# peleiden/rl-rubiks

Hardware: AMD Instinct MI355X
Metric: MCTS node expansions/sec, depth-20 scrambles (higher is better)
Workload: dtype f32 (f16x3 split: three f16 MFMA products per layer, fp32 accumulate); 1 GPU; 1024 depth-20 MCTS trees/GPU, c=0.6, graph search, max_states 175000, pool 8x1024, fc_small weights/fc_small_r1; trees_per_gpu=1024, max_states=175000, scramble_depth=20, parallelism=scramble-sharded x1

## Files before the change

rl-rubiks_amd/csrc/rubiks_net.hip:

```cpp
#include <atomic>

#include <type_traits>

#include "rubiks_common.h"
#include "rubiks_netmath.h"

namespace rubiks {

constexpr int kOH = 480;

__device__ __forceinline__ float act_apply(float x, int act, float alpha) {
    if (act == RC_ACT_RELU) return fmaxf(x, 0.f);
    if (act == RC_ACT_ELU) return x > 0.f ? x : alpha * (__expf(x) - 1.f);
    return x;
}


typedef __attribute__((ext_vector_type(8))) __bf16 bf16x8;
typedef __attribute__((ext_vector_type(8))) _Float16 f16x8;
typedef __attribute__((ext_vector_type(16))) float f32x16;

constexpr int kMfCols = 128;
constexpr int kMfPitch = 976;
constexpr int kMfWaves = 8;
constexpr int kMfTile = 32;
constexpr int kMfSub = 1;

template <int ACT, bool F16>
__global__ __launch_bounds__(kMfWaves * kWave) void k_first_layer_mfma(const u8 *__restrict__ soa, size_t n, size_t stride,
                                                                     const uint4 *__restrict__ w1, const float *__restrict__ bias,
                                                                     uint4 *__restrict__ out, u32 H, u32 rows_per_block,
                                                                     float alpha) {
    extern __shared__ __attribute__((aligned(256))) unsigned char lds[];
    unsigned char *wslice = lds;
    const u32 tid = threadIdx.x, wave = tid >> 6, lane = tid & 63;
    uint4 *onehot = reinterpret_cast<uint4 *>(lds + kMfCols * kMfPitch);
    const u32 col_tiles = H / kMfCols;
    const u32 ct = blockIdx.x % col_tiles, rg = blockIdx.x / col_tiles;
    const size_t row_lo = (size_t)rg * rows_per_block;
    if (row_lo >= n) return;
    const size_t row_hi = (row_lo + rows_per_block < n) ? row_lo + rows_per_block : n;

    {
        constexpr int kPer = kMfCols * 60 / (kMfWaves * kWave), kBatch = 5;
#pragma unroll
        for (int b0 = 0; b0 < kPer; b0 += kBatch) {
            uint4 tmp[kBatch];
#pragma unroll
            for (int t = 0; t < kBatch; ++t) {
                const u32 i = tid + (b0 + t) * (kMfWaves * kWave);
                tmp[t] = w1[(size_t)(ct * kMfCols + i / 60) * 60 + i % 60];
            }
#pragma unroll
            for (int t = 0; t < kBatch; ++t) {
                const u32 i = tid + (b0 + t) * (kMfWaves * kWave);
                const u32 g = i / 60, slot = (g & 3) * 32 + (g >> 2);
                *reinterpret_cast<uint4 *>(wslice + slot * kMfPitch + (i % 60) * 16) = tmp[t];
            }
        }
    }
    if (tid < 9) {
        u32 w[4] = {0, 0, 0, 0};
        const u32 one = F16 ? 0x3c00u : 0x3f80u;
        if (tid < 8) w[tid >> 1] = (tid & 1) ? one << 16 : one;
        onehot[tid] = make_uint4(w[0], w[1], w[2], w[3]);
    }
    const u32 r = lane & 31, h = lane >> 5;
    float b[4];
#pragma unroll
    for (int c = 0; c < 4; ++c) b[c] = bias[ct * kMfCols + 4 * r + c];
    __syncthreads();

    const u32 off_a = h ? 8u : 0u, off_c = h ? 16u : 8u;
    constexpr size_t kStep = (size_t)kMfWaves * kMfSub * kMfTile;
    for (size_t t0 = row_lo + (size_t)wave * kMfSub * kMfTile; t0 < row_hi; t0 += kStep) {
        u32 pk[kMfSub][5];
#pragma unroll
        for (int u = 0; u < kMfSub; ++u) {
            const size_t row = t0 + (size_t)u * kMfTile + r;
            const u8 *p = soa + (row < n ? row : n - 1);
            u32 raw[kPlanes];
#pragma unroll
            for (int j = 0; j < kPlanes; ++j) raw[j] = p[(size_t)j * stride];
#pragma unroll
            for (int q = 0; q < 5; ++q)
                pk[u][q] = (raw[4 * q] & 31u) | (raw[4 * q + 1] & 31u) << 8 | (raw[4 * q + 2] & 31u) << 16 | (raw[4 * q + 3] & 31u) << 24;
        }
        auto code = [&](int u, int j) -> u32 { return (pk[u][j >> 2] >> (8 * (j & 3))) & 0xffu; };
        f32x16 acc[kMfSub][4];
#pragma unroll
        for (int u = 0; u < kMfSub; ++u)
#pragma unroll
            for (int c = 0; c < 4; ++c)
#pragma unroll
                for (int i = 0; i < 16; ++i) acc[u][c][i] = b[c];
        auto a_frag = [&](int u, int ks) -> uint4 {
            const int m2 = ks / 3, ph = ks % 3;
            const u32 pos = ph == 0 ? code(u, 2 * m2) - off_a : ph == 1 ? (h ? code(u, 2 * m2 + 1) : code(u, 2 * m2) - 16u)
                                                                         : code(u, 2 * m2 + 1) - off_c;
            return onehot[min(pos, 8u)];
        };
        const unsigned char *bbase = wslice + r * kMfPitch + 16 * h;
        uint4 a_cur[kMfSub], b_cur[4];
#pragma unroll
        for (int u = 0; u < kMfSub; ++u) a_cur[u] = a_frag(u, 0);
#pragma unroll
        for (int c = 0; c < 4; ++c) b_cur[c] = *reinterpret_cast<const uint4 *>(bbase + c * 32 * kMfPitch);
#pragma unroll
        for (int ks = 0; ks < 30; ++ks) {
            uint4 a_nxt[kMfSub], b_nxt[4] = {b_cur[0], b_cur[1], b_cur[2], b_cur[3]};
#pragma unroll
            for (int u = 0; u < kMfSub; ++u) a_nxt[u] = a_cur[u];
            if (ks + 1 < 30) {
#pragma unroll
                for (int c = 0; c < 4; ++c) b_nxt[c] = *reinterpret_cast<const uint4 *>(bbase + c * 32 * kMfPitch + 32 * (ks + 1));
#pragma unroll
                for (int u = 0; u < kMfSub; ++u) a_nxt[u] = a_frag(u, ks + 1);
            }
            __builtin_amdgcn_sched_barrier(0);
#pragma unroll
            for (int c = 0; c < 4; ++c)
#pragma unroll
                for (int u = 0; u < kMfSub; ++u) {
                    if (F16)
                        acc[u][c] = __builtin_amdgcn_mfma_f32_32x32x16_f16(__builtin_bit_cast(f16x8, a_cur[u]),
                                                                           __builtin_bit_cast(f16x8, b_cur[c]), acc[u][c], 0, 0, 0);
                    else
                        acc[u][c] = __builtin_amdgcn_mfma_f32_32x32x16_bf16(__builtin_bit_cast(bf16x8, a_cur[u]),
                                                                            __builtin_bit_cast(bf16x8, b_cur[c]), acc[u][c], 0, 0, 0);
                }
            __builtin_amdgcn_sched_barrier(0);
#pragma unroll
            for (int u = 0; u < kMfSub; ++u) a_cur[u] = a_nxt[u];
#pragma unroll
            for (int c = 0; c < 4; ++c) b_cur[c] = b_nxt[c];
        }
        uint2 *out2 = reinterpret_cast<uint2 *>(out);
#pragma unroll
        for (int u = 0; u < kMfSub; ++u)
#pragma unroll
            for (int i = 0; i < 16; ++i) {
                const size_t row = t0 + (size_t)u * kMfTile + (i & 3) + 8 * (i >> 2) + 4 * h;
                const uint2 v = make_uint2(pack_bf16(act_apply(acc[u][0][i], ACT, alpha), act_apply(acc[u][1][i], ACT, alpha)),
                                           pack_bf16(act_apply(acc[u][2][i], ACT, alpha), act_apply(acc[u][3][i], ACT, alpha)));
                if (row < n) out2[row * (H / 4) + ct * (kMfCols / 4) + r] = v;
            }
    }
}

typedef __attribute__((ext_vector_type(4))) float f32x4;
constexpr int kHeadK = 1024, kHeadSteps = kHeadK / 32, kHeadMaxOut = 16;

// ... 360 lines not shown
__global__ __launch_bounds__(kMfWaves * kWave) void k_first_layer_split(const u8 *__restrict__ soa, size_t n, size_t stride,
                                                                      const uint4 *__restrict__ w_hi, const uint4 *__restrict__ w_lo,
                                                                      const float *__restrict__ bias, u32 *__restrict__ out, u32 H,
                                                                      u32 rows_per_block, float alpha, int *__restrict__ range_flag) {
    extern __shared__ __attribute__((aligned(256))) unsigned char lds[];
    constexpr int kTables = 2;
    bool out_of_range = false;
    unsigned char *wslice = lds;
    const u32 tid = threadIdx.x, lane = tid & 63;
    const u32 wave = __builtin_amdgcn_readfirstlane(tid >> 6);
    uint4 *onehot = reinterpret_cast<uint4 *>(lds + kTables * kSpCols * kMfPitch);
    const u32 col_tiles = H / kSpCols;
    const u32 ct = blockIdx.x % col_tiles, rg = blockIdx.x / col_tiles;
    const size_t row_lo = (size_t)rg * rows_per_block;
    if (row_lo >= n) return;
    const size_t row_hi = (row_lo + rows_per_block < n) ? row_lo + rows_per_block : n;
    {
        constexpr int kBatch = 5, kPer = kTables * kSpCols * 60 / (kMfWaves * kWave) / kBatch * kBatch;
#pragma unroll
        for (int b0 = 0; b0 < kPer; b0 += kBatch) {
            uint4 tmp[kBatch];
#pragma unroll
            for (int t = 0; t < kBatch; ++t) {
                const u32 i = tid + (b0 + t) * (kMfWaves * kWave), tbl = i / (kSpCols * 60), j = i % (kSpCols * 60);
                tmp[t] = (tbl ? w_lo : w_hi)[(size_t)(ct * kSpCols + j / 60) * 60 + j % 60];
            }
#pragma unroll
            for (int t = 0; t < kBatch; ++t) {
                const u32 i = tid + (b0 + t) * (kMfWaves * kWave), tbl = i / (kSpCols * 60), j = i % (kSpCols * 60);
                const u32 g = j / 60, slot = (g & 1) * 32 + (g >> 1);
                *reinterpret_cast<uint4 *>(wslice + (tbl * kSpCols + slot) * kMfPitch + (j % 60) * 16) = tmp[t];
            }
        }
        static_assert(kPer * kMfWaves * kWave == kTables * kSpCols * 60, "the staging loop covers the slices exactly");
    }
    if (tid < 9 * kTables) {
        u32 w[4] = {0, 0, 0, 0};
        const u32 p = tid % 9, one = tid < 9 ? kHalfOne : kHalfScaleInv;
        if (p < 8) w[p >> 1] = (p & 1) ? one << 16 : one;
        onehot[tid] = make_uint4(w[0], w[1], w[2], w[3]);
    }
    const u32 r = lane & 31, h = lane >> 5;
    float b[2];
#pragma unroll
    for (int c = 0; c < 2; ++c) b[c] = bias[ct * kSpCols + 2 * r + c];
    __syncthreads();

    const u32 off_a = h ? 8u : 0u, off_c = h ? 16u : 8u;
    constexpr size_t kStep = (size_t)kMfWaves * kSpSub * kMfTile;
    const u32 n_pass = (u32)((row_hi - row_lo + kStep - 1) / kStep);
    for (u32 pass = 0; pass < n_pass; ++pass) {
        const size_t t0 = row_lo + (size_t)pass * kStep + (size_t)wave * kSpSub * kMfTile;
        if (t0 >= row_hi) break;
        u32 pk[kSpSub][5];
#pragma unroll
        for (int u = 0; u < kSpSub; ++u) {
            const size_t row = t0 + (size_t)u * kMfTile + r;
            const u8 *p = soa + (row < n ? row : n - 1);
            u32 raw[kPlanes];
#pragma unroll
            for (int j = 0; j < kPlanes; ++j) raw[j] = p[(size_t)j * stride];
#pragma unroll
            for (int q = 0; q < 5; ++q)
                pk[u][q] = (raw[4 * q] & 31u) | (raw[4 * q + 1] & 31u) << 8 | (raw[4 * q + 2] & 31u) << 16 | (raw[4 * q + 3] & 31u) << 24;
        }
        auto code = [&](int u, int j) -> u32 { return (pk[u][j >> 2] >> (8 * (j & 3))) & 0xffu; };
        f32x16 acc[kSpSub][2];
#pragma unroll
        for (int u = 0; u < kSpSub; ++u)
#pragma unroll
            for (int c = 0; c < 2; ++c)
#pragma unroll
                for (int i = 0; i < 16; ++i) acc[u][c][i] = b[c];
#pragma unroll 1
        for (int tbl = 0; tbl < kTables; ++tbl) {
            const uint4 *frag = onehot + 9 * tbl;
            const unsigned char *bbase = wslice + ((size_t)tbl * kSpCols + r) * kMfPitch + 16 * h;
            auto a_frag = [&](int u, int ks) -> uint4 {
                const int m2 = ks / 3, ph = ks % 3;
                const u32 pos = ph == 0 ? code(u, 2 * m2) - off_a : ph == 1 ? (h ? code(u, 2 * m2 + 1) : code(u, 2 * m2) - 16u)
                                                                             : code(u, 2 * m2 + 1) - off_c;
                return frag[min(pos, 8u)];
            };
            uint4 a_cur[kSpSub], b_cur[2];
#pragma unroll
            for (int u = 0; u < kSpSub; ++u) a_cur[u] = a_frag(u, 0);
#pragma unroll
            for (int c = 0; c < 2; ++c) b_cur[c] = *reinterpret_cast<const uint4 *>(bbase + c * 32 * kMfPitch);
#pragma unroll
            for (int ks = 0; ks < 30; ++ks) {
                uint4 a_nxt[kSpSub], b_nxt[2] = {b_cur[0], b_cur[1]};
#pragma unroll
                for (int u = 0; u < kSpSub; ++u) a_nxt[u] = a_cur[u];
                if (ks + 1 < 30) {
#pragma unroll
                    for (int c = 0; c < 2; ++c) b_nxt[c] = *reinterpret_cast<const uint4 *>(bbase + c * 32 * kMfPitch + 32 * (ks + 1));
#pragma unroll
                    for (int u = 0; u < kSpSub; ++u) a_nxt[u] = a_frag(u, ks + 1);
                }
                __builtin_amdgcn_sched_barrier(0);
#pragma unroll
                for (int c = 0; c < 2; ++c)
#pragma unroll
                    for (int u = 0; u < kSpSub; ++u)
                        acc[u][c] = __builtin_amdgcn_mfma_f32_32x32x16_f16(__builtin_bit_cast(f16x8, a_cur[u]),
                                                                           __builtin_bit_cast(f16x8, b_cur[c]), acc[u][c], 0, 0, 0);
                __builtin_amdgcn_sched_barrier(0);
#pragma unroll
                for (int u = 0; u < kSpSub; ++u) a_cur[u] = a_nxt[u];
#pragma unroll
                for (int c = 0; c < 2; ++c) b_cur[c] = b_nxt[c];
            }
        }
        const size_t lim = row_hi < n ? row_hi : n;
        u32 *o_hi = out + t0 * (size_t)H + (ct * kSpCols) / 2;
        u32 *o_lo = o_hi + H / 2;
        if (t0 + (size_t)kSpSub * kMfTile <= lim) {
            u32 off = 4 * h * H + r;
#pragma unroll
            for (int u = 0; u < kSpSub; ++u)
#pragma unroll
                for (int i = 0; i < 16; ++i) {
                    const float y0 = act_value<ACT>(acc[u][0][i], alpha), y1 = act_value<ACT>(acc[u][1][i], alpha);
                    out_of_range |= !(fabsf(y0) <= 65504.0f) || !(fabsf(y1) <= 65504.0f);
                    const SplitPair sp = split_pair(y0, y1);
                    o_hi[off] = sp.hi;
                    o_lo[off] = sp.lo;
                    off += ((i & 3) == 3 ? 5u : 1u) * H;
                }
        } else {
#pragma unroll
            for (int u = 0; u < kSpSub; ++u)
#pragma unroll
                for (int i = 0; i < 16; ++i) {
                    const size_t row = t0 + (size_t)u * kMfTile + (i & 3) + 8 * (i >> 2) + 4 * h;
                    const float y0 = act_value<ACT>(acc[u][0][i], alpha), y1 = act_value<ACT>(acc[u][1][i], alpha);
                    if (row < lim) {
                        out_of_range |= !(fabsf(y0) <= 65504.0f) || !(fabsf(y1) <= 65504.0f);
                        const SplitPair sp = split_pair(y0, y1);
                        u32 *orow = out + row * H;
                        orow[(ct * kSpCols) / 2 + r] = sp.hi;
                        orow[H / 2 + (ct * kSpCols) / 2 + r] = sp.lo;
                    }
                }
        }
    }
    if (range_flag && out_of_range) atomicOr(range_flag, 1);
}

constexpr int kGaCols = 64, kGaRows = 480;
#ifndef RUBIKS_GATHER_ABLATE
#define RUBIKS_GATHER_ABLATE 0
#endif
typedef float f32x2 __attribute__((ext_vector_type(2)));

template <int ACT, int WAVES, int C, bool MAP = false>
__global__ __launch_bounds__(WAVES * kWave) void k_first_layer_gather(const u8 *__restrict__ soa, size_t n, size_t stride,
                                                                     const float4 *__restrict__ w_rows, const float *__restrict__ bias,
                                                                     unsigned char *__restrict__ out, u32 H, u32 rows_per_block, float alpha,
                                                                     int *__restrict__ range_flag, const u32 *__restrict__ rows_dev,
                                                                     const int *__restrict__ src_map) {
    static_assert(C == 4 || C == 8, "4 or 8 columns per lane");
    constexpr int R = C / 4;
    constexpr u32 kLanes = kGaCols / C;
    constexpr u32 kStates = kWave / kLanes;
    extern __shared__ __attribute__((aligned(256))) unsigned char lds[];
    const u32 tid = threadIdx.x, lane = tid & 63;
    const u32 wave = __builtin_amdgcn_readfirstlane(tid >> 6);
    const u32 col_tiles = H / kGaCols, ct = blockIdx.x % col_tiles, rg = blockIdx.x / col_tiles;
    const u32 last_state = (u32)(n - 1);
    if (MAP) {
        n = min((size_t)*rows_dev, n);
        const u32 per_group = (u32)ceil_div(n, (size_t)(gridDim.x / col_tiles)), unit = per_group < WAVES * kStates ? kStates : WAVES * kStates;
        rows_per_block = (per_group + unit - 1) / unit * unit;
    }
    const size_t row_lo = (size_t)rg * rows_per_block;
    if (row_lo >= n) return;
    const size_t row_hi = (row_lo + rows_per_block < n) ? row_lo + rows_per_block : n;
    {
        constexpr u32 kChunks = kGaRows * (kGaCols / 4), kThreads = WAVES * kWave, kBatch = 4;
        for (u32 i0 = tid; i0 < kChunks; i0 += kBatch * kThreads) {
            float4 tmp[kBatch];
#pragma unroll
            for (u32 b = 0; b < kBatch; ++b) {
                const u32 i = i0 + b * kThreads;
                if (i < kChunks) tmp[b] = w_rows[(size_t)(i >> 4) * (H / 4) + ct * (kGaCols / 4) + (i & 15)];
            }
#pragma unroll
            for (u32 b = 0; b < kBatch; ++b) {
                const u32 i = i0 + b * kThreads;
                if (i < kChunks) reinterpret_cast<float4 *>(lds)[i] = tmp[b];
            }
        }
    }
    const u32 u = lane % kLanes, sub = lane / kLanes;
    const u32 col = ct * kGaCols + C * u;
    float4 b4[R];
#pragma unroll
    for (int r = 0; r < R; ++r) b4[r] = *reinterpret_cast<const float4 *>(bias + col + 4 * r);
    bool out_of_range = false;
    const __amdgpu_buffer_rsrc_t planes = __builtin_amdgcn_make_buffer_rsrc((void *)soa, 0, (int)(u32)(kPlanes * stride), 0x00020000);
    const u32 last = (u32)(n - 1), pitch = (u32)stride;
    auto codes_of = [&](size_t t, u32 (&c)[kPlanes]) {
        u32 tv = t < n ? (u32)t : last;
        if (MAP) tv = min((u32)src_map[tv], last_state);
#pragma unroll
        for (int j = 0; j < kPlanes; ++j) c[j] = (RUBIKS_GATHER_ABLATE & 4) ? (tv + j) % 24u : (u32)__builtin_amdgcn_raw_buffer_load_b8(planes, tv, (u32)j * pitch, 0);
    };
    const u32 base0 = u * (4 * C), base1 = u * (4 * C) + 11 * 24 * (kGaCols * 4);
    __syncthreads();
    constexpr size_t kStep = (size_t)WAVES * kStates;
    size_t t = row_lo + (size_t)wave * kStates + sub;
    u32 code[kPlanes], code_next[kPlanes];
    codes_of(t, code);
    for (size_t t0 = row_lo + (size_t)wave * kStates; t0 < row_hi; t0 += kStep, t += kStep) {
        const bool more = t0 + kStep < row_hi;
        f32x2 acc[2 * R];
#pragma unroll
        for (int r = 0; r < R; ++r) acc[2 * r] = f32x2{b4[r].x, b4[r].y}, acc[2 * r + 1] = f32x2{b4[r].z, b4[r].w};
        constexpr int kBatch = 10 / R;
#pragma unroll
        for (int part = 0; part < kPlanes / kBatch; ++part) {
            float4 v[kBatch][R];
#pragma unroll
            for (int i = 0; i < kBatch; ++i) {
                const int j = part * kBatch + i;
                const u32 at = (code[j] << 8) + (j < 11 ? base0 : base1);
                const unsigned char *rowp = lds + at + (j < 11 ? j : j - 11) * 24 * (kGaCols * 4);
#pragma unroll
                for (int r = 0; r < R; ++r)
                    v[i][r] = (RUBIKS_GATHER_ABLATE & 2) ? make_float4(__uint_as_float(at), 1.f, 2.f, 3.f) : *reinterpret_cast<const float4 *>(rowp + 16 * r);
            }
            __builtin_amdgcn_sched_barrier(0);
            if (part == 0 && more) codes_of(t + kStep, code_next);
            __builtin_amdgcn_sched_barrier(0);
#pragma unroll
            for (int i = 0; i < kBatch; ++i)
#pragma unroll
                for (int r = 0; r < R; ++r) {
                    acc[2 * r] += f32x2{v[i][r].x, v[i][r].y};
                    acc[2 * r + 1] += f32x2{v[i][r].z, v[i][r].w};
                }
            __builtin_amdgcn_sched_barrier(0);
        }
        bool bad = false;
        SplitPair sp[2 * R];
#pragma unroll
        for (int p = 0; p < 2 * R; ++p) {
            if (!(RUBIKS_GATHER_ABLATE & 8)) acc[p] = act_value2<ACT>(acc[p], alpha);
            bad |= !(fabsf(acc[p].x) <= 65504.0f);
            bad |= !(fabsf(acc[p].y) <= 65504.0f);
            sp[p] = split_pair(acc[p].x, acc[p].y);
        }
        const bool live = (RUBIKS_GATHER_ABLATE & 1) ? (t < row_hi && acc[0].x == 1.2345e-30f) : t < row_hi;
        unsigned char *orow = out + t * ((size_t)H * 4);
        if (C == 8) {
            if (live) {
                out_of_range |= bad;
                *reinterpret_cast<uint4 *>(orow + (size_t)col * 2) = make_uint4(sp[0].hi, sp[1].hi, sp[2 * R - 2].hi, sp[2 * R - 1].hi);
                *reinterpret_cast<uint4 *>(orow + ((size_t)H + col) * 2) = make_uint4(sp[0].lo, sp[1].lo, sp[2 * R - 2].lo, sp[2 * R - 1].lo);
            }
        } else {
            constexpr int kSwapPairs = 0xB1;
            const u32 n_hi0 = (u32)__builtin_amdgcn_mov_dpp((int)sp[0].hi, kSwapPairs, 0xF, 0xF, true), n_hi1 = (u32)__builtin_amdgcn_mov_dpp((int)sp[1].hi, kSwapPairs, 0xF, 0xF, true);
            const u32 n_lo0 = (u32)__builtin_amdgcn_mov_dpp((int)sp[0].lo, kSwapPairs, 0xF, 0xF, true), n_lo1 = (u32)__builtin_amdgcn_mov_dpp((int)sp[1].lo, kSwapPairs, 0xF, 0xF, true);
            if (live) {
                out_of_range |= bad;
                const bool odd = lane & 1u;
                const uint4 both = odd ? make_uint4(n_lo0, n_lo1, sp[0].lo, sp[1].lo) : make_uint4(sp[0].hi, sp[1].hi, n_hi0, n_hi1);
                *reinterpret_cast<uint4 *>(orow + (odd ? (size_t)H + col - 4 : (size_t)col) * 2) = both;
            }
        }
        if (more) {
#pragma unroll
            for (int j = 0; j < kPlanes; ++j) code[j] = code_next[j];
        }
    }
    if (range_flag && out_of_range) atomicOr(range_flag, 1);
}

extern "C" int rc_oh_split_f16(const int8_t *soa, size_t n, size_t stride, uint16_t *out, rc_stream_t stream) {
    if (n == 0) return RC_OK;
    RC_CHECK_SOA(soa, n, stride);
    RC_REQUIRE(out != nullptr, RC_ERR_NULL);
    RC_REQUIRE(aligned16(out), RC_ERR_ALIGN);
    hipLaunchKernelGGL(k_oh_split_f16, dim3(grid_for(n * (2 * kOH / 8), kBlock, 256 * 16)), dim3(kBlock), 0, (hipStream_t)stream,
                       (const u8 *)soa, n, stride, (uint4 *)out);
    return launch_status();
}

extern "C" int rc_split_act_f16(const float *c, const float *c_corr, float corr_scale, size_t n_rows, size_t n_cols, const float *bias,
                                int activation, float alpha, uint16_t *out_hi_lo, float *out_f32, rc_stream_t stream) {
    if (n_rows == 0 || n_cols == 0) return RC_OK;
    RC_REQUIRE(c && bias && (out_hi_lo || out_f32), RC_ERR_NULL);
    RC_REQUIRE(aligned16(c) && aligned16(c_corr) && aligned16(bias) && aligned16(out_hi_lo) && aligned16(out_f32) && n_cols % 8 == 0, RC_ERR_ALIGN);
    RC_REQUIRE(activation >= RC_ACT_NONE && activation <= RC_ACT_ELU, RC_ERR_RANGE);
    const dim3 grid(grid_for(n_rows * (n_cols / 8), kBlock, 256 * 16)), block(kBlock);
    hipStream_t s = (hipStream_t)stream;
#define RC_LAUNCH_SPLIT(ACT)                                                                                                  \
    hipLaunchKernelGGL(k_split_act<ACT>, grid, block, 0, s, (const float4 *)c, (const float4 *)c_corr, corr_scale, n_rows, n_cols, \
                       (const float4 *)bias, alpha,                                                                            \
                       (uint4 *)out_hi_lo, (float4 *)out_f32)
    if (activation == RC_ACT_ELU) RC_LAUNCH_SPLIT(RC_ACT_ELU);
    else if (activation == RC_ACT_RELU) RC_LAUNCH_SPLIT(RC_ACT_RELU);
    else RC_LAUNCH_SPLIT(RC_ACT_NONE);
#undef RC_LAUNCH_SPLIT
    return launch_status();
}

static int split_reduce(const float *partials, size_t partial_stride, int n_partials, int n_corr, size_t n_rows, size_t n_cols,
                        const float *bias, const uint16_t *residual_hi_lo, int activation, float alpha, const float *post_scale,
                        const float *post_shift, uint16_t *out_hi_lo, float *out_f32, int32_t *range_flag, const uint32_t *rows_dev,
                        rc_stream_t stream) {
    if (n_rows == 0 || n_cols == 0) return RC_OK;
    RC_REQUIRE(partials && bias && (out_hi_lo || out_f32), RC_ERR_NULL);
    RC_REQUIRE((post_scale == nullptr) == (post_shift == nullptr), RC_ERR_NULL);
    RC_REQUIRE(aligned16(partials) && aligned16(bias) && aligned16(residual_hi_lo) && aligned16(post_scale) && aligned16(post_shift) &&
                   aligned16(out_hi_lo) && aligned16(out_f32) && n_cols % 8 == 0 && partial_stride % 4 == 0, RC_ERR_ALIGN);
    RC_REQUIRE(activation >= RC_ACT_NONE && activation <= RC_ACT_ELU && n_partials >= 1 && n_partials <= 64 && n_corr >= 0 &&
                   n_corr <= n_partials && (n_partials == 1 || partial_stride >= n_rows * n_cols), RC_ERR_RANGE);
    const dim3 grid(grid_for(n_rows * (n_cols / 8), kBlock, 256 * 16)), block(kBlock);
    hipStream_t s = (hipStream_t)stream;
#define RC_LAUNCH_RED(ACT)                                                                                                       \
    hipLaunchKernelGGL(k_split_reduce<ACT>, grid, block, 0, s, (const float4 *)partials, partial_stride / 4, n_partials, n_corr, n_rows, \
                       n_cols, (const float4 *)bias, (const uint4 *)residual_hi_lo, alpha, (const float4 *)post_scale,                \
                       (const float4 *)post_shift, (uint4 *)out_hi_lo, (float4 *)out_f32, (int *)range_flag, rows_dev)
    if (activation == RC_ACT_ELU) RC_LAUNCH_RED(RC_ACT_ELU);
    else if (activation == RC_ACT_RELU) RC_LAUNCH_RED(RC_ACT_RELU);
    else RC_LAUNCH_RED(RC_ACT_NONE);
#undef RC_LAUNCH_RED
    return launch_status();
}

extern "C" int rc_split_reduce_f16(const float *partials, size_t partial_stride, int n_partials, int n_corr, size_t n_rows, size_t n_cols,
                                   const float *bias, const uint16_t *residual_hi_lo, int activation, float alpha, const float *post_scale,
                                   const float *post_shift, uint16_t *out_hi_lo, float *out_f32, int32_t *range_flag, rc_stream_t stream) {
    return split_reduce(partials, partial_stride, n_partials, n_corr, n_rows, n_cols, bias, residual_hi_lo, activation, alpha, post_scale,
                        post_shift, out_hi_lo, out_f32, range_flag, nullptr, stream);
}

extern "C" int rc_split_reduce_rows_f16(const float *partials, size_t partial_stride, int n_partials, int n_corr, size_t n_rows, size_t n_cols,
                                        const float *bias, const uint16_t *residual_hi_lo, int activation, float alpha,
                                        const float *post_scale, const float *post_shift, uint16_t *out_hi_lo, float *out_f32,
                                        int32_t *range_flag, const uint32_t *rows_dev, rc_stream_t stream) {
    RC_REQUIRE(rows_dev != nullptr, RC_ERR_NULL);
    return split_reduce(partials, partial_stride, n_partials, n_corr, n_rows, n_cols, bias, residual_hi_lo, activation, alpha, post_scale,
                        post_shift, out_hi_lo, out_f32, range_flag, rows_dev, stream);
}

static int head_split(const float *c, const float *c_corr, float corr_scale, size_t n, size_t K, const float *bias_h, int activation,
                      float alpha, const float *w, const float *bias_o, size_t n_out, float *out, const uint32_t *rows_dev,
                      const int32_t *src_map, rc_stream_t stream) {
    if (n == 0) return RC_OK;
    RC_REQUIRE(c && bias_h && w && bias_o && out && (rows_dev == nullptr) == (src_map == nullptr), RC_ERR_NULL);
    RC_REQUIRE(aligned16(c) && aligned16(c_corr) && aligned16(bias_h) && aligned16(w), RC_ERR_ALIGN);
    RC_REQUIRE((K == 512 || K == 1024) && n_out >= 1 && n_out <= (size_t)kHeadMaxOut && activation >= RC_ACT_NONE && activation <= RC_ACT_ELU,
               RC_ERR_RANGE);
    const unsigned grid = grid_for(ceil_div(n, (size_t)16) * kBlock, kBlock, 256 * 4);
    hipStream_t s = (hipStream_t)stream;
#define RC_LAUNCH_HS(ACT, KB, MAP)                                                                                             \
    hipLaunchKernelGGL((k_head_split<ACT, KB, MAP>), dim3(grid), dim3(kBlock), 0, s, (const float4 *)c, (const float4 *)c_corr, corr_scale, \
                       n, (const float4 *)bias_h, alpha, (const float4 *)w, bias_o, (u32)n_out, out, rows_dev, src_map)
#define RC_LAUNCH_HS_K(ACT)                                     \
    do {                                                        \
        if (rows_dev) {                                         \
            if (K == 1024) RC_LAUNCH_HS(ACT, 16, true);         \
            else RC_LAUNCH_HS(ACT, 8, true);                    \
        } else if (K == 1024) RC_LAUNCH_HS(ACT, 16, false);     \
        else RC_LAUNCH_HS(ACT, 8, false);                       \
    } while (0)
    if (activation == RC_ACT_ELU) RC_LAUNCH_HS_K(RC_ACT_ELU);
    else if (activation == RC_ACT_RELU) RC_LAUNCH_HS_K(RC_ACT_RELU);
    else RC_LAUNCH_HS_K(RC_ACT_NONE);
#undef RC_LAUNCH_HS_K
#undef RC_LAUNCH_HS
    return launch_status();
}

extern "C" int rc_head_split_f32(const float *c, const float *c_corr, float corr_scale, size_t n, size_t K, const float *bias_h,
                                 int activation, float alpha, const float *w, const float *bias_o, size_t n_out, float *out,
                                 rc_stream_t stream) {
    return head_split(c, c_corr, corr_scale, n, K, bias_h, activation, alpha, w, bias_o, n_out, out, nullptr, nullptr, stream);
}

extern "C" int rc_head_split_rows_f32(const float *c, const float *c_corr, float corr_scale, size_t n, size_t K, const float *bias_h,
                                      int activation, float alpha, const float *w, const float *bias_o, size_t n_out, float *out,
                                      const uint32_t *rows_dev, const int32_t *src_map, rc_stream_t stream) {
    RC_REQUIRE(rows_dev && src_map, RC_ERR_NULL);
    return head_split(c, c_corr, corr_scale, n, K, bias_h, activation, alpha, w, bias_o, n_out, out, rows_dev, src_map, stream);
}

extern "C" int rc_first_layer_split_f16(const int8_t *soa, size_t n, size_t stride, const uint16_t *w_hi, const uint16_t *w_lo,
                                        const float *bias, uint16_t *out_hi_lo, size_t H, int activation, float alpha,
                                        rc_stream_t stream) {
    return rc_first_layer_split_flag_f16(soa, n, stride, w_hi, w_lo, bias, out_hi_lo, H, activation, alpha, nullptr, stream);
}

extern "C" int rc_first_layer_split_flag_f16(const int8_t *soa, size_t n, size_t stride, const uint16_t *w_hi, const uint16_t *w_lo,
                                             const float *bias, uint16_t *out_hi_lo, size_t H, int activation, float alpha,
                                             int32_t *range_flag, rc_stream_t stream) {
    if (n == 0) return RC_OK;
    RC_CHECK_SOA(soa, n, stride);
    RC_REQUIRE(w_hi && w_lo && bias && out_hi_lo, RC_ERR_NULL);
    RC_REQUIRE(aligned16(w_hi) && aligned16(w_lo) && aligned16(out_hi_lo), RC_ERR_ALIGN);
    RC_REQUIRE(H >= (size_t)kSpCols && H % kSpCols == 0 && activation >= RC_ACT_NONE && activation <= RC_ACT_ELU, RC_ERR_RANGE);
    const u32 col_tiles = (u32)(H / kSpCols);
    u32 row_groups = (256 + col_tiles - 1) / col_tiles;
    constexpr u32 kRowsPerPass = kMfWaves * kSpSub * kMfTile;
    const size_t per_group = ceil_div(n, row_groups);
    u32 rows_per_block = (u32)round_up(per_group, per_group < kRowsPerPass ? (size_t)kSpSub * kMfTile : (size_t)kRowsPerPass);
    row_groups = (u32)ceil_div(n, rows_per_block);
    const size_t lds_bytes = (size_t)2 * kSpCols * kMfPitch + 2 * 9 * 16;
    const dim3 grid(col_tiles * row_groups), block(kMfWaves * kWave);
    hipStream_t s = (hipStream_t)stream;
#define RC_LAUNCH_SP(ACT)                                                                                             \
    do {                                                                                                              \
        static std::atomic<unsigned long long> attr_set{0};                                                           \
        int dev_ = 0;                                                                                                 \
        (void)hipGetDevice(&dev_);                                                                                    \
        if (!((attr_set.load(std::memory_order_acquire) >> (dev_ & 63)) & 1ull)) {                                     \
            hipError_t e = hipFuncSetAttribute((const void *)k_first_layer_split<ACT>, hipFuncAttributeMaxDynamicSharedMemorySize, \
                                               (int)lds_bytes);                                                       \
            if (e != hipSuccess) return hip_rc(e);                                                                    \
            attr_set.fetch_or(1ull << (dev_ & 63), std::memory_order_release);                                        \
        }                                                                                                             \
        hipLaunchKernelGGL((k_first_layer_split<ACT>), grid, block, lds_bytes, s, (const u8 *)soa, n, stride, (const uint4 *)w_hi, \
                           (const uint4 *)w_lo, bias, (u32 *)out_hi_lo, (u32)H, rows_per_block, alpha, (int *)range_flag); \
    } while (0)
    if (activation == RC_ACT_ELU) RC_LAUNCH_SP(RC_ACT_ELU);
    else if (activation == RC_ACT_RELU) RC_LAUNCH_SP(RC_ACT_RELU);
    else RC_LAUNCH_SP(RC_ACT_NONE);
#undef RC_LAUNCH_SP
    return launch_status();
}

static int first_layer_gather(const int8_t *soa, size_t n, size_t stride, const float *w_rows, const float *bias, uint16_t *out_hi_lo,
                              size_t H, int activation, float alpha, int32_t *range_flag, const uint32_t *rows_dev, const int32_t *src_map,
                              int form, rc_stream_t stream) {
    if (n == 0) return RC_OK;
    RC_CHECK_SOA(soa, n, stride);
    RC_REQUIRE(w_rows && bias && out_hi_lo && (rows_dev == nullptr) == (src_map == nullptr), RC_ERR_NULL);
    RC_REQUIRE(form >= 0 && form <= 2, RC_ERR_RANGE);
    RC_REQUIRE(aligned16(w_rows) && aligned16(bias) && aligned16(out_hi_lo), RC_ERR_ALIGN);
    RC_REQUIRE(H >= (size_t)kGaCols && H % kGaCols == 0 && H < (1u << 24) && activation >= RC_ACT_NONE && activation <= RC_ACT_ELU, RC_ERR_RANGE);
    RC_REQUIRE(stride * kPlanes < (1ull << 32), RC_ERR_RANGE);
    const u32 col_tiles = (u32)(H / kGaCols);
    const size_t lds_bytes = (size_t)kGaRows * kGaCols * 4;
    hipStream_t s = (hipStream_t)stream;
    const bool wide = form ? form == 2 : n * col_tiles > (size_t)5000 * 64;
    const u32 waves = wide ? 8 : 16, states = wide ? 8 : 4;
    u32 row_groups = (256 + col_tiles - 1) / col_tiles;
    const u32 rows_per_pass = waves * states;
    const size_t per_group = ceil_div(n, (size_t)row_groups);
    const u32 rows_per_block = (u32)round_up(per_group, per_group < rows_per_pass ? (size_t)states : (size_t)rows_per_pass);
    row_groups = (u32)ceil_div(n, (size_t)rows_per_block);
    const dim3 grid(col_tiles * row_groups);
#define RC_LAUNCH_GA(ACT, WAVES, C, MAP)                                                                                 \
    do {                                                                                                              \
        static std::atomic<unsigned long long> attr_set{0};                                                           \
        int dev_ = 0;                                                                                                 \
        (void)hipGetDevice(&dev_);                                                                                    \
        if (!((attr_set.load(std::memory_order_acquire) >> (dev_ & 63)) & 1ull)) {                                     \
            hipError_t e = hipFuncSetAttribute((const void *)k_first_layer_gather<ACT, WAVES, C, MAP>,                \
                                               hipFuncAttributeMaxDynamicSharedMemorySize, (int)lds_bytes);           \
            if (e != hipSuccess) return hip_rc(e);                                                                    \
            attr_set.fetch_or(1ull << (dev_ & 63), std::memory_order_release);                                        \
        }                                                                                                             \
        hipLaunchKernelGGL((k_first_layer_gather<ACT, WAVES, C, MAP>), grid, dim3(WAVES * kWave), lds_bytes, s, (const u8 *)soa, n, stride, \
                           (const float4 *)w_rows, bias, (unsigned char *)out_hi_lo, (u32)H, rows_per_block, alpha, (int *)range_flag,  \
                           rows_dev, src_map);                                                                          \
    } while (0)
#define RC_LAUNCH_GA_ACT(ACT)                              \
    do {                                                   \
        if (rows_dev) {                                    \
            if (wide) RC_LAUNCH_GA(ACT, 8, 8, true);       \
            else RC_LAUNCH_GA(ACT, 16, 4, true);           \
        } else if (wide) RC_LAUNCH_GA(ACT, 8, 8, false);   \
        else RC_LAUNCH_GA(ACT, 16, 4, false);              \
    } while (0)
    if (activation == RC_ACT_ELU) RC_LAUNCH_GA_ACT(RC_ACT_ELU);
    else if (activation == RC_ACT_RELU) RC_LAUNCH_GA_ACT(RC_ACT_RELU);
    else RC_LAUNCH_GA_ACT(RC_ACT_NONE);
#undef RC_LAUNCH_GA_ACT
#undef RC_LAUNCH_GA
    return launch_status();
}

extern "C" int rc_first_layer_gather_f16(const int8_t *soa, size_t n, size_t stride, const float *w_rows, const float *bias,
                                         uint16_t *out_hi_lo, size_t H, int activation, float alpha, int32_t *range_flag,
                                         rc_stream_t stream) {
    return first_layer_gather(soa, n, stride, w_rows, bias, out_hi_lo, H, activation, alpha, range_flag, nullptr, nullptr, 0, stream);
}

extern "C" int rc_first_layer_gather_rows_f16(const int8_t *soa, size_t n, size_t stride, const float *w_rows, const float *bias,
                                              uint16_t *out_hi_lo, size_t H, int activation, float alpha, int32_t *range_flag,
                                              const uint32_t *rows_dev, const int32_t *src_map, int form, rc_stream_t stream) {
    return first_layer_gather(soa, n, stride, w_rows, bias, out_hi_lo, H, activation, alpha, range_flag, rows_dev, src_map, form, stream);
}

extern "C" int rc_adi_targets(const float *values, const uint8_t *child_solved, const uint8_t *state_solved, size_t n,
                              size_t depth, float win_reward, int fix_mode, int64_t *policy_target, float *value_target,
                              rc_stream_t stream) {
    if (n == 0) return RC_OK;
    RC_REQUIRE(values && child_solved && policy_target && value_target, RC_ERR_NULL);
    RC_REQUIRE(fix_mode >= 0 && fix_mode <= 2 && depth > 0, RC_ERR_RANGE);
    RC_REQUIRE(fix_mode != 1 || state_solved != nullptr, RC_ERR_NULL);
    hipLaunchKernelGGL(k_adi_targets, dim3(grid_for(n)), dim3(kBlock), 0, (hipStream_t)stream, values, child_solved,
                       state_solved, n, depth, win_reward, fix_mode, (long long *)policy_target, value_target);
    return launch_status();
}
```

Baseline: 14.17 million node expansions/s.

## Software-pipeline the wide first-layer gather across passes with triple-buffered codes

Rewrites the C==8 path of the first-layer gather kernel. Cubie codes are fetched two passes ahead through a rotating set of three code buffers, and the first LDS row reads of the next pass overlap the current accumulation. Lanes are remapped so each lane reads two 16-byte slices and swaps halves via DPP, allowing a single buffer store per output half. The wide launch also moves from 8 to 12 waves, and the weight staging loop is restructured to unroll fully. This aims to hide global code-load and LDS latency, at the cost of more registers and higher occupancy pressure.

```diff
diff --git a/rl-rubiks_amd/csrc/rubiks_net.hip b/rl-rubiks_amd/csrc/rubiks_net.hip
--- a/rl-rubiks_amd/csrc/rubiks_net.hip
+++ b/rl-rubiks_amd/csrc/rubiks_net.hip
@@ -1,3 +1,4 @@
+#include <utility>
 #include <atomic>
 
 #include <type_traits>
@@ -664,7 +665,26 @@
 #ifndef RUBIKS_GATHER_ABLATE
 #define RUBIKS_GATHER_ABLATE 0
 #endif
+constexpr int kGaWideWaves = 12, kGaAhead = 4;
 typedef float f32x2 __attribute__((ext_vector_type(2)));
+typedef float f32x4 __attribute__((ext_vector_type(4)));
+typedef u32 u32x4 __attribute__((ext_vector_type(4)));
+#define RC_GA_PLANES(X) X(0) X(1) X(2) X(3) X(4) X(5) X(6) X(7) X(8) X(9) X(10) X(11) X(12) X(13) X(14) X(15) X(16) X(17) X(18) X(19)
+struct GaCodes {
+#define RC_GA_FIELD(j) u32 c##j;
+    RC_GA_PLANES(RC_GA_FIELD)
+#undef RC_GA_FIELD
+    template <int J> __device__ __forceinline__ u32 &at() {
+        static_assert(J >= 0 && J < kPlanes, "one code per cubie");
+#define RC_GA_PICK(j) if constexpr (J == j) return c##j; else
+        RC_GA_PLANES(RC_GA_PICK) return c0;
+#undef RC_GA_PICK
+    }
+    template <int J> __device__ __forceinline__ u32 at() const { return const_cast<GaCodes *>(this)->template at<J>(); }
+};
+#define RC_INLINE __attribute__((always_inline))
+template <class F, int... I> __device__ __forceinline__ void static_for_each(F &&f, std::integer_sequence<int, I...>) { (f(std::integral_constant<int, I>{}), ...); }
+template <int N, class F> __device__ __forceinline__ void static_for(F &&f) { static_for_each(f, std::make_integer_sequence<int, N>{}); }
 
 template <int ACT, int WAVES, int C, bool MAP = false>
 __global__ __launch_bounds__(WAVES * kWave) void k_first_layer_gather(const u8 *__restrict__ soa, size_t n, size_t stride,
@@ -673,7 +693,6 @@
                                                                      int *__restrict__ range_flag, const u32 *__restrict__ rows_dev,
                                                                      const int *__restrict__ src_map) {
     static_assert(C == 4 || C == 8, "4 or 8 columns per lane");
-    constexpr int R = C / 4;
     constexpr u32 kLanes = kGaCols / C;
     constexpr u32 kStates = kWave / kLanes;
     extern __shared__ __attribute__((aligned(256))) unsigned char lds[];
@@ -690,89 +709,185 @@
     if (row_lo >= n) return;
     const size_t row_hi = (row_lo + rows_per_block < n) ? row_lo + rows_per_block : n;
     {
-        constexpr u32 kChunks = kGaRows * (kGaCols / 4), kThreads = WAVES * kWave, kBatch = 4;
-        for (u32 i0 = tid; i0 < kChunks; i0 += kBatch * kThreads) {
+        constexpr u32 kChunks = kGaRows * (kGaCols / 4), kThreads = WAVES * kWave, kRounds = kChunks / kThreads, kBatch = 5;
+        const float4 *src = w_rows + ct * (kGaCols / 4);
+        const auto chunk = [&](u32 i) { return src[(size_t)(i >> 4) * (H / 4) + (i & 15)]; };
+#pragma unroll
+        for (u32 r0 = 0; r0 < kRounds; r0 += kBatch) {
             float4 tmp[kBatch];
 #pragma unroll
-            for (u32 b = 0; b < kBatch; ++b) {
-                const u32 i = i0 + b * kThreads;
-                if (i < kChunks) tmp[b] = w_rows[(size_t)(i >> 4) * (H / 4) + ct * (kGaCols / 4) + (i & 15)];
-            }
-#pragma unroll
-            for (u32 b = 0; b < kBatch; ++b) {
-                const u32 i = i0 + b * kThreads;
-                if (i < kChunks) reinterpret_cast<float4 *>(lds)[i] = tmp[b];
-            }
-        }
+            for (u32 b = 0; b < kBatch; ++b)
+                if (r0 + b < kRounds) tmp[b] = chunk(tid + (r0 + b) * kThreads);
+#pragma unroll
+            for (u32 b = 0; b < kBatch; ++b)
+                if (r0 + b < kRounds) reinterpret_cast<float4 *>(lds)[tid + (r0 + b) * kThreads] = tmp[b];
+        }
+        if (kChunks % kThreads != 0 && tid < kChunks % kThreads) reinterpret_cast<float4 *>(lds)[tid + kRounds * kThreads] = chunk(tid + kRounds * kThreads);
     }
     const u32 u = lane % kLanes, sub = lane / kLanes;
-    const u32 col = ct * kGaCols + C * u;
-    float4 b4[R];
-#pragma unroll
-    for (int r = 0; r < R; ++r) b4[r] = *reinterpret_cast<const float4 *>(bias + col + 4 * r);
     bool out_of_range = false;
-    const __amdgpu_buffer_rsrc_t planes = __builtin_amdgcn_make_buffer_rsrc((void *)soa, 0, (int)(u32)(kPlanes * stride), 0x00020000);
-    const u32 last = (u32)(n - 1), pitch = (u32)stride;
-    auto codes_of = [&](size_t t, u32 (&c)[kPlanes]) {
-        u32 tv = t < n ? (u32)t : last;
-        if (MAP) tv = min((u32)src_map[tv], last_state);
-#pragma unroll
-        for (int j = 0; j < kPlanes; ++j) c[j] = (RUBIKS_GATHER_ABLATE & 4) ? (tv + j) % 24u : (u32)__builtin_amdgcn_raw_buffer_load_b8(planes, tv, (u32)j * pitch, 0);
-    };
-    const u32 base0 = u * (4 * C), base1 = u * (4 * C) + 11 * 24 * (kGaCols * 4);
-    __syncthreads();
+    const u32 last = (u32)(n - 1);
     constexpr size_t kStep = (size_t)WAVES * kStates;
     size_t t = row_lo + (size_t)wave * kStates + sub;
-    u32 code[kPlanes], code_next[kPlanes];
-    codes_of(t, code);
-    for (size_t t0 = row_lo + (size_t)wave * kStates; t0 < row_hi; t0 += kStep, t += kStep) {
-        const bool more = t0 + kStep < row_hi;
-        f32x2 acc[2 * R];
-#pragma unroll
-        for (int r = 0; r < R; ++r) acc[2 * r] = f32x2{b4[r].x, b4[r].y}, acc[2 * r + 1] = f32x2{b4[r].z, b4[r].w};
-        constexpr int kBatch = 10 / R;
-#pragma unroll
-        for (int part = 0; part < kPlanes / kBatch; ++part) {
-            float4 v[kBatch][R];
-#pragma unroll
-            for (int i = 0; i < kBatch; ++i) {
-                const int j = part * kBatch + i;
-                const u32 at = (code[j] << 8) + (j < 11 ? base0 : base1);
-                const unsigned char *rowp = lds + at + (j < 11 ? j : j - 11) * 24 * (kGaCols * 4);
-#pragma unroll
-                for (int r = 0; r < R; ++r)
-                    v[i][r] = (RUBIKS_GATHER_ABLATE & 2) ? make_float4(__uint_as_float(at), 1.f, 2.f, 3.f) : *reinterpret_cast<const float4 *>(rowp + 16 * r);
-            }
-            __builtin_amdgcn_sched_barrier(0);
-            if (part == 0 && more) codes_of(t + kStep, code_next);
-            __builtin_amdgcn_sched_barrier(0);
-#pragma unroll
-            for (int i = 0; i < kBatch; ++i)
-#pragma unroll
-                for (int r = 0; r < R; ++r) {
-                    acc[2 * r] += f32x2{v[i][r].x, v[i][r].y};
-                    acc[2 * r + 1] += f32x2{v[i][r].z, v[i][r].w};
+    if constexpr (C == 8) {
+        constexpr int kAhead = kGaAhead;
+        const u32 p = (u ^ sub) & 1u, slot = u ^ (8u * p);
+        const u32 lane0 = 16u * slot;
+        const u32 col_k = ct * kGaCols + 4 * slot, col_s = ct * kGaCols + 4 * (slot ^ 8u);
+        const float4 bias_k = *reinterpret_cast<const float4 *>(bias + col_k), bias_s = *reinterpret_cast<const float4 *>(bias + col_s);
+        const u32 row_bytes = H * 4, out_at = sub * row_bytes + (ct * kGaCols + 32u * p + 4u * (u & 6u)) * 2;
+        const bool odd = u & 1u;
+        const auto row_of = [&](size_t ahead) RC_INLINE {
+            const size_t tt = t + ahead * kStep;
+            return tt < n ? (u32)tt : last;
+        };
+        const auto request = [&](u32 tv, GaCodes &c) RC_INLINE {
+            static_for<kPlanes>([&](auto jc) RC_INLINE {
+                constexpr int j = decltype(jc)::value;
+                c.template at<j>() = (RUBIKS_GATHER_ABLATE & 4) ? (tv + j) % 24u : (u32)(soa + (size_t)j * stride)[tv];
+            });
+        };
+        typedef const f32x4 __attribute__((address_space(3))) *SliceRow;
+        u32 first0 = (u32)(size_t)(__attribute__((address_space(3))) unsigned char *)lds + lane0, first1 = first0 + 11 * 24 * (kGaCols * 4);
+        u32 to_second = (lane0 ^ 128u) - lane0;
+        asm("" : "+v"(first0), "+v"(first1), "+v"(to_second));
+        const auto read_row = [&](const GaCodes &c, auto jc, f32x4(&v)[2]) RC_INLINE {
+            constexpr int j = decltype(jc)::value;
+            constexpr u32 imm = (u32)(j < 11 ? j : j - 11) * 24 * (kGaCols * 4);
+            u32 at0 = (c.template at<j>() << 8) + (j < 11 ? first0 : first1);
+            asm("" : "+v"(at0));
+            u32 at1 = at0 + to_second;
+            asm("" : "+v"(at1));
+            if (RUBIKS_GATHER_ABLATE & 2) {
+                v[0] = v[1] = f32x4{__uint_as_float(at0 + at1), 1.f, 2.f, 3.f};
+            } else {
+                v[0] = *(SliceRow)(size_t)(at0 + imm);
+                v[1] = *(SliceRow)(size_t)(at1 + imm);
+            }
+        };
+        const bool any = row_lo + (size_t)wave * kStates < row_hi;
+        GaCodes code_a, code_b, code_c;
+        u32 map_next = 0;
+        if (any) {
+            if (MAP) {
+                request(min((u32)src_map[row_of(0)], last_state), code_a);
+                request(min((u32)src_map[row_of(1)], last_state), code_b);
+                map_next = (u32)src_map[row_of(2)];
+            } else {
+                request(row_of(0), code_a);
+                request(row_of(1), code_b);
+            }
+        }
+        __syncthreads();
+        if (!any) return;
+        f32x4 head[kAhead][2];
+        static_for<kAhead>([&](auto ic) RC_INLINE { read_row(code_a, ic, head[decltype(ic)::value]); });
+        size_t t0 = row_lo + (size_t)wave * kStates;
+        const auto pass = [&](const GaCodes &cur, const GaCodes &nxt, GaCodes &far) RC_INLINE {
+            if (MAP) {
+                const u32 state = min(map_next, last_state);
+                map_next = (u32)src_map[row_of(3)];
+                request(state, far);
+            } else {
+                request(row_of(2), far);
+            }
+            f32x2 acc[4] = {f32x2{bias_k.x, bias_k.y}, f32x2{bias_k.z, bias_k.w}, f32x2{bias_s.x, bias_s.y}, f32x2{bias_s.z, bias_s.w}};
+            f32x4 v[kPlanes + kAhead][2];
+#pragma unroll
+            for (int i = 0; i < kAhead; ++i) v[i][0] = head[i][0], v[i][1] = head[i][1];
+            static_for<kPlanes>([&](auto jc) RC_INLINE {
+                constexpr int j = decltype(jc)::value, ja = j + kAhead;
+                if constexpr (ja < kPlanes) read_row(cur, std::integral_constant<int, ja>{}, v[ja]);
+                else read_row(nxt, std::integral_constant<int, ja - kPlanes>{}, v[ja]);
+                __builtin_amdgcn_sched_barrier(0);
+                acc[0] += v[j][0].xy;
+                acc[1] += v[j][0].zw;
+                acc[2] += v[j][1].xy;
+                acc[3] += v[j][1].zw;
+                __builtin_amdgcn_sched_barrier(0);
+            });
+#pragma unroll
+            for (int i = 0; i < kAhead; ++i) head[i][0] = v[kPlanes + i][0], head[i][1] = v[kPlanes + i][1];
+            bool bad = false;
+            SplitPair sp[4];
+#pragma unroll
+            for (int q = 0; q < 4; ++q) {
+                if (!(RUBIKS_GATHER_ABLATE & 8)) acc[q] = act_value2<ACT>(acc[q], alpha);
+                bad |= !(fabsf(acc[q].x) <= 65504.0f);
+                bad |= !(fabsf(acc[q].y) <= 65504.0f);
+                sp[q] = split_pair(acc[q].x, acc[q].y);
+            }
+            constexpr int kSwapPairs = 0xB1;
+            const u32 n_hi0 = (u32)__builtin_amdgcn_mov_dpp((int)sp[2].hi, kSwapPairs, 0xF, 0xF, true), n_hi1 = (u32)__builtin_amdgcn_mov_dpp((int)sp[3].hi, kSwapPairs, 0xF, 0xF, true);
+            const u32 n_lo0 = (u32)__builtin_amdgcn_mov_dpp((int)sp[2].lo, kSwapPairs, 0xF, 0xF, true), n_lo1 = (u32)__builtin_amdgcn_mov_dpp((int)sp[3].lo, kSwapPairs, 0xF, 0xF, true);
+            const u32 rows = (RUBIKS_GATHER_ABLATE & 1) ? 0u : t0 < row_hi ? (u32)min(row_hi - t0, (size_t)kStates) : 0u;
+            const __amdgpu_buffer_rsrc_t pass_rows = __builtin_amdgcn_make_buffer_rsrc(out + t0 * ((size_t)H * 4), 0, (int)(rows * row_bytes), 0x00020000);
+            out_of_range |= bad && sub < rows;
+            const u32x4 his = odd ? u32x4{n_hi0, n_hi1, sp[0].hi, sp[1].hi} : u32x4{sp[0].hi, sp[1].hi, n_hi0, n_hi1};
+            const u32x4 los = odd ? u32x4{n_lo0, n_lo1, sp[0].lo, sp[1].lo} : u32x4{sp[0].lo, sp[1].lo, n_lo0, n_lo1};
+            __builtin_amdgcn_raw_buffer_store_b128(his, pass_rows, out_at, 0, 0);
+            __builtin_amdgcn_raw_buffer_store_b128(los, pass_rows, out_at, row_bytes / 2, 0);
+            t0 += kStep, t += kStep;
+        };
+        size_t passes = (row_hi - t0 + kStep - 1) / kStep;
+        for (; passes >= 3; passes -= 3) {
+            pass(code_a, code_b, code_c);
+            pass(code_b, code_c, code_a);
+            pass(code_c, code_a, code_b);
+        }
+        if (passes >= 1) pass(code_a, code_b, code_c);
+        if (passes == 2) pass(code_b, code_c, code_a);
+        if (range_flag && out_of_range) atomicOr(range_flag, 1);
+    } else {
+        const u32 col = ct * kGaCols + 4 * u;
+        const float4 b4 = *reinterpret_cast<const float4 *>(bias + col);
+        const __amdgpu_buffer_rsrc_t planes = __builtin_amdgcn_make_buffer_rsrc((void *)soa, 0, (int)(u32)(kPlanes * stride), 0x00020000);
+        const u32 pitch = (u32)stride;
+        auto codes_of = [&](size_t t, u32 (&c)[kPlanes]) {
+            u32 tv = t < n ? (u32)t : last;
+            if (MAP) tv = min((u32)src_map[tv], last_state);
+#pragma unroll
+            for (int j = 0; j < kPlanes; ++j) c[j] = (RUBIKS_GATHER_ABLATE & 4) ? (tv + j) % 24u : (u32)__builtin_amdgcn_raw_buffer_load_b8(planes, tv, (u32)j * pitch, 0);
+        };
+        const u32 base0 = u * 16, base1 = u * 16 + 11 * 24 * (kGaCols * 4);
+        __syncthreads();
+        u32 code[kPlanes], code_next[kPlanes];
+        codes_of(t, code);
+        for (size_t t0 = row_lo + (size_t)wave * kStates; t0 < row_hi; t0 += kStep, t += kStep) {
+            const bool more = t0 + kStep < row_hi;
+            f32x2 acc[2] = {f32x2{b4.x, b4.y}, f32x2{b4.z, b4.w}};
+            constexpr int kBatch = 10;
+#pragma unroll
+            for (int part = 0; part < kPlanes / kBatch; ++part) {
+                float4 v[kBatch];
+#pragma unroll
+                for (int i = 0; i < kBatch; ++i) {
+                    const int j = part * kBatch + i;
+                    const u32 at = (code[j] << 8) + (j < 11 ? base0 : base1);
+                    const unsigned char *rowp = lds + at + (j < 11 ? j : j - 11) * 24 * (kGaCols * 4);
+                    v[i] = (RUBIKS_GATHER_ABLATE & 2) ? make_float4(__uint_as_float(at), 1.f, 2.f, 3.f) : *reinterpret_cast<const float4 *>(rowp);
                 }
-            __builtin_amdgcn_sched_barrier(0);
-        }
-        bool bad = false;
-        SplitPair sp[2 * R];
-#pragma unroll
-        for (int p = 0; p < 2 * R; ++p) {
-            if (!(RUBIKS_GATHER_ABLATE & 8)) acc[p] = act_value2<ACT>(acc[p], alpha);
-            bad |= !(fabsf(acc[p].x) <= 65504.0f);
-            bad |= !(fabsf(acc[p].y) <= 65504.0f);
-            sp[p] = split_pair(acc[p].x, acc[p].y);
-        }
-        const bool live = (RUBIKS_GATHER_ABLATE & 1) ? (t < row_hi && acc[0].x == 1.2345e-30f) : t < row_hi;
-        unsigned char *orow = out + t * ((size_t)H * 4);
-        if (C == 8) {
-            if (live) {
-                out_of_range |= bad;
-                *reinterpret_cast<uint4 *>(orow + (size_t)col * 2) = make_uint4(sp[0].hi, sp[1].hi, sp[2 * R - 2].hi, sp[2 * R - 1].hi);
-                *reinterpret_cast<uint4 *>(orow + ((size_t)H + col) * 2) = make_uint4(sp[0].lo, sp[1].lo, sp[2 * R - 2].lo, sp[2 * R - 1].lo);
-            }
-        } else {
+                __builtin_amdgcn_sched_barrier(0);
+                if (part == 0 && more) codes_of(t + kStep, code_next);
+                __builtin_amdgcn_sched_barrier(0);
+#pragma unroll
+                for (int i = 0; i < kBatch; ++i) {
+                    acc[0] += f32x2{v[i].x, v[i].y};
+                    acc[1] += f32x2{v[i].z, v[i].w};
+                }
+                __builtin_amdgcn_sched_barrier(0);
+            }
+            bool bad = false;
+            SplitPair sp[2];
+#pragma unroll
+            for (int p = 0; p < 2; ++p) {
+                if (!(RUBIKS_GATHER_ABLATE & 8)) acc[p] = act_value2<ACT>(acc[p], alpha);
+                bad |= !(fabsf(acc[p].x) <= 65504.0f);
+                bad |= !(fabsf(acc[p].y) <= 65504.0f);
+                sp[p] = split_pair(acc[p].x, acc[p].y);
+            }
+            const bool live = (RUBIKS_GATHER_ABLATE & 1) ? (t < row_hi && acc[0].x == 1.2345e-30f) : t < row_hi;
+            unsigned char *orow = out + t * ((size_t)H * 4);
             constexpr int kSwapPairs = 0xB1;
             const u32 n_hi0 = (u32)__builtin_amdgcn_mov_dpp((int)sp[0].hi, kSwapPairs, 0xF, 0xF, true), n_hi1 = (u32)__builtin_amdgcn_mov_dpp((int)sp[1].hi, kSwapPairs, 0xF, 0xF, true);
             const u32 n_lo0 = (u32)__builtin_amdgcn_mov_dpp((int)sp[0].lo, kSwapPairs, 0xF, 0xF, true), n_lo1 = (u32)__builtin_amdgcn_mov_dpp((int)sp[1].lo, kSwapPairs, 0xF, 0xF, true);
@@ -782,13 +897,13 @@
                 const uint4 both = odd ? make_uint4(n_lo0, n_lo1, sp[0].lo, sp[1].lo) : make_uint4(sp[0].hi, sp[1].hi, n_hi0, n_hi1);
                 *reinterpret_cast<uint4 *>(orow + (odd ? (size_t)H + col - 4 : (size_t)col) * 2) = both;
             }
-        }
-        if (more) {
-#pragma unroll
-            for (int j = 0; j < kPlanes; ++j) code[j] = code_next[j];
-        }
-    }
-    if (range_flag && out_of_range) atomicOr(range_flag, 1);
+            if (more) {
+#pragma unroll
+                for (int j = 0; j < kPlanes; ++j) code[j] = code_next[j];
+            }
+        }
+        if (range_flag && out_of_range) atomicOr(range_flag, 1);
+    }
 }
 
 extern "C" int rc_oh_split_f16(const int8_t *soa, size_t n, size_t stride, uint16_t *out, rc_stream_t stream) {
@@ -960,7 +1075,7 @@
     const size_t lds_bytes = (size_t)kGaRows * kGaCols * 4;
     hipStream_t s = (hipStream_t)stream;
     const bool wide = form ? form == 2 : n * col_tiles > (size_t)5000 * 64;
-    const u32 waves = wide ? 8 : 16, states = wide ? 8 : 4;
+    const u32 waves = wide ? kGaWideWaves : 16, states = wide ? 8 : 4;
     u32 row_groups = (256 + col_tiles - 1) / col_tiles;
     const u32 rows_per_pass = waves * states;
     const size_t per_group = ceil_div(n, (size_t)row_groups);
@@ -985,9 +1100,9 @@
 #define RC_LAUNCH_GA_ACT(ACT)                              \
     do {                                                   \
         if (rows_dev) {                                    \
-            if (wide) RC_LAUNCH_GA(ACT, 8, 8, true);       \
+            if (wide) RC_LAUNCH_GA(ACT, kGaWideWaves, 8, true);      \
             else RC_LAUNCH_GA(ACT, 16, 4, true);           \
-        } else if (wide) RC_LAUNCH_GA(ACT, 8, 8, false);   \
+        } else if (wide) RC_LAUNCH_GA(ACT, kGaWideWaves, 8, false);  \
         else RC_LAUNCH_GA(ACT, 16, 4, false);              \
     } while (0)
     if (activation == RC_ACT_ELU) RC_LAUNCH_GA_ACT(RC_ACT_ELU);
```

New measurement: 14.48 million node expansions/s (median of 6 runs). +2.2%, better.
